# TianmingQiu/BNN_KFAC

Measured on AMD Instinct MI355X. Metric: images/sec for full KFAC factor pass + factor inversion, MNIST MLP, 1/2/4/8 GPUs, higher is better.
Workload: dtype f32; 1 GPU; C2: MLP 784-128-10 KFAC factor pass over 60000 images/rank (batch 4096/rank, global batch 4096) + invert(0.04000000000000001, 200); global_batch=4096, images_per_rank=60000, parallelism=dp1

## Files before the change

### bnn_kfac_amd/_native.py

```python
from __future__ import annotations

import atexit
import ctypes
import os
import threading

import torch

_HERE = os.path.dirname(os.path.abspath(__file__))
LIB_PATH = os.environ.get("BNN_KFAC_AMD_LIB", os.path.join(_HERE, "libkfac_hip.so"))

KFAC_OK, KFAC_EINVAL, KFAC_ELAUNCH, KFAC_EWORKSPACE = 0, -1, -2, -3
ROWMAJOR, CHANNEL, PATCH = 0, 1, 2
OUT_INV_CHOL, OUT_INVERSE = 0, 1
TRI_SYMMETRIC, TRI_LOWER = 0, 1
(PROF_FACTOR_TILES, PROF_FACTOR_REDUCE, PROF_INVERT, PROF_QUAD_TILES, PROF_FACTOR_SYRK3,
 PROF_FACTOR_X3, PROF_FACTOR_CONV, PROF_FACTOR_CHANNEL_SMALL, PROF_SYEV, PROF_FACTOR_CONV_X3,
 PROF_FACTOR_CONV_X3S, PROF_FACTOR_CONV_X3F, PROF_FACTOR_CHANNEL_X3) = range(13)
PROF_FACTOR_KERNELS = {PROF_FACTOR_TILES: "kfac_factor_tiles", PROF_FACTOR_SYRK3: "kfac_factor_syrk3",
                       PROF_FACTOR_X3: "kfac_factor_tiles_x3", PROF_FACTOR_CONV: "kfac_factor_conv",
                       PROF_FACTOR_CHANNEL_SMALL: "kfac_factor_channel_small",
                       PROF_FACTOR_CONV_X3: "kfac_factor_conv_x3", PROF_FACTOR_CONV_X3S: "kfac_factor_conv_x3s",
                       PROF_FACTOR_CONV_X3F: "kfac_factor_conv_x3f", PROF_FACTOR_CHANNEL_X3: "kfac_factor_channel_x3"}

# ... 74 lines not shown


class CovOuterFullJob(ctypes.Structure):
    _fields_ = [("a", c_vp), ("lda", c_i64), ("cols", c_i32), ("has_ones", c_i32), ("D", c_vp),
                ("ldD", c_i64), ("nG", c_i32), ("reserved", c_i32), ("VA", c_vp), ("ldA", c_i64),
                ("VG", c_vp), ("ldG", c_i64), ("W", c_vp), ("ldW", c_i64)]


class InfCovJob(ctypes.Structure):
    _fields_ = [("J", c_vp), ("ldJ", c_i64), ("nA", c_i32), ("nG", c_i32), ("UA", c_vp),
                ("ldA", c_i64), ("ra", c_i32), ("UG", c_vp), ("ldG", c_i64), ("rg", c_i32),
                ("W", c_vp), ("ldW", c_i64), ("F", c_vp), ("ldF", c_i64)]


class InfCovOuterJob(ctypes.Structure):
    _fields_ = [("a", c_vp), ("lda", c_i64), ("cols", c_i32), ("has_ones", c_i32), ("D", c_vp),
                ("ldD", c_i64), ("nG", c_i32), ("reserved", c_i32), ("UA", c_vp), ("ldA", c_i64),
                ("ra", c_i32), ("UG", c_vp), ("ldG", c_i64), ("rg", c_i32), ("W", c_vp),
                ("ldW", c_i64), ("F", c_vp), ("ldF", c_i64)]


class SampleJob(ctypes.Structure):
    _fields_ = [("LA", c_vp), ("ldA", c_i64), ("LG", c_vp), ("ldG", c_i64), ("Z", c_vp),
                ("nA", c_i32), ("nG", c_i32), ("W", c_vp), ("ldW", c_i64), ("bias", c_vp),
                ("wcols", c_i32), ("dense", c_i32)]


class EfbJob(ctypes.Structure):
    _fields_ = [("VA", c_vp), ("ldA", c_i64), ("VG", c_vp), ("ldG", c_i64), ("grad", c_vp),
                ("ld_grad", c_i64), ("state", c_vp), ("ld_state", c_i64), ("diag", c_vp),
                ("ld_diag", c_i64), ("nA", c_i32), ("nG", c_i32), ("accumulate", c_i32),
                ("scale", c_f32)]


class GramJob(ctypes.Structure):
    _fields_ = [("UA", c_vp), ("ldA", c_i64), ("UG", c_vp), ("ldG", c_i64), ("c", c_vp),
                ("sigma", c_vp), ("out", c_vp), ("ldo", c_i64), ("nA", c_i32), ("nG", c_i32),
                ("la", c_i32), ("lg", c_i32)]


class TriJob(ctypes.Structure):
    _fields_ = [("F", c_vp), ("ldF", c_i64), ("n", c_i32), ("reserved", c_i32), ("offset", c_i64)]


SIGNATURES = {
    "kfac_factor_workspace_bytes": (ctypes.c_size_t, [ctypes.POINTER(FactorJob), ctypes.c_int]),
    "kfac_factor_update": (ctypes.c_int, [ctypes.POINTER(FactorJob), ctypes.c_int, c_vp,
                                          ctypes.c_size_t, c_vp]),
    "kfac_factor_accum_plan": (ctypes.c_int, [ctypes.POINTER(FactorJob), ctypes.c_int,
                                              ctypes.POINTER(c_i32), ctypes.POINTER(ctypes.c_size_t)]),
    "kfac_factor_route": (ctypes.c_int, [ctypes.POINTER(FactorJob), ctypes.c_int, ctypes.POINTER(c_i32)]),
    "kfac_factor_flush": (ctypes.c_int, [ctypes.POINTER(FactorJob), ctypes.c_int, c_vp]),
    "kfac_x3_unit_table": (ctypes.c_int, [ctypes.c_int, ctypes.POINTER(c_i32), ctypes.c_int]),
    "kfac_syrk_linear": (ctypes.c_int, [c_vp, c_i64, c_i64, c_i64, ctypes.c_int, c_f32, c_f32,
                                        c_vp, c_i64, c_vp, ctypes.c_size_t, c_vp]),
    "kfac_syrk_conv": (ctypes.c_int, [c_vp, c_i64] + [ctypes.c_int] * 10 + [c_f32, c_f32, c_vp,
                                                                            c_i64, c_vp,
                                                                            ctypes.c_size_t, c_vp]),
    "kfac_syrk_convgrad": (ctypes.c_int, [c_vp, c_i64, ctypes.c_int, c_i64, c_f32, c_f32, c_vp,
                                          c_i64, c_vp, ctypes.c_size_t, c_vp]),
    "kfac_invert_workspace_bytes": (ctypes.c_size_t, [ctypes.POINTER(InvertJob), ctypes.c_int]),
    "kfac_invert": (ctypes.c_int, [ctypes.POINTER(InvertJob), ctypes.c_int, c_vp,
                                   ctypes.c_size_t, c_vp, c_vp]),
    "kfac_invert_ex": (ctypes.c_int, [ctypes.POINTER(InvertJob), ctypes.c_int, c_vp,
                                      ctypes.c_size_t, c_vp, c_vp, c_vp]),
    "kfac_damped_inv_chol": (ctypes.c_int, [c_vp, ctypes.c_int, c_i64, c_f64, c_f64, c_vp, c_i64,
                                            c_vp, ctypes.c_size_t, c_vp, c_vp]),
    "kfac_eig_workspace_bytes": (ctypes.c_size_t, [ctypes.POINTER(EigJob), ctypes.c_int]),
    "kfac_syev": (ctypes.c_int, [ctypes.POINTER(EigJob), ctypes.c_int, c_vp, ctypes.c_size_t,
                                 c_vp, c_vp]),
    "kfac_quadform_workspace_bytes": (ctypes.c_size_t, [ctypes.POINTER(QuadJob), ctypes.c_int,
                                                        c_i64]),
    "kfac_kron_quadform": (ctypes.c_int, [ctypes.POINTER(QuadJob), ctypes.c_int, c_i64,
                                          ctypes.c_int, c_vp, c_vp, ctypes.c_size_t, c_vp]),
    "kfac_kron_cov_workspace_bytes": (ctypes.c_size_t, [ctypes.POINTER(CovJob), ctypes.c_int, c_i64,
                                                        ctypes.c_int]),
    "kfac_kron_cov": (ctypes.c_int, [ctypes.POINTER(CovJob), ctypes.c_int, c_i64, ctypes.c_int,
                                     ctypes.c_int, c_vp, c_vp, ctypes.c_size_t, c_vp]),
    "kfac_kron_cov_outer_workspace_bytes": (ctypes.c_size_t, [ctypes.POINTER(CovOuterJob), ctypes.c_int,
                                                              c_i64, ctypes.c_int]),
    "kfac_kron_cov_outer": (ctypes.c_int, [ctypes.POINTER(CovOuterJob), ctypes.c_int, c_i64, ctypes.c_int,
                                           ctypes.c_int, c_vp, c_vp, ctypes.c_size_t, c_vp]),
    "kfac_cov_conv_rows": (ctypes.c_int, [ctypes.POINTER(CovConvRowsJob), ctypes.c_int, c_i64, ctypes.c_int,
                                          c_vp]),
    "kfac_kron_cov_joint_workspace_bytes": (ctypes.c_size_t, [ctypes.POINTER(CovJob), ctypes.c_int, c_i64,
                                                              ctypes.c_int]),
    "kfac_kron_cov_joint": (ctypes.c_int, [ctypes.POINTER(CovJob), ctypes.c_int, c_i64, ctypes.c_int,
                                           ctypes.c_int, c_vp, c_i64, c_vp, ctypes.c_size_t, c_vp]),
    "kfac_kron_cov_outer_joint_workspace_bytes": (ctypes.c_size_t, [ctypes.POINTER(CovOuterJob),
                                                                    ctypes.c_int, c_i64, ctypes.c_int]),
    "kfac_kron_cov_outer_joint": (ctypes.c_int, [ctypes.POINTER(CovOuterJob), ctypes.c_int, c_i64,
                                                 ctypes.c_int, ctypes.c_int, c_vp, c_i64, c_vp,
                                                 ctypes.c_size_t, c_vp]),
    "kfac_kron_cov_tiled_workspace_bytes": (ctypes.c_size_t, [ctypes.POINTER(CovJob), ctypes.c_int, c_i64,
                                                              ctypes.c_int]),
    "kfac_kron_cov_tiled": (ctypes.c_int, [ctypes.POINTER(CovJob), ctypes.c_int, c_i64, ctypes.c_int,
                                           ctypes.c_int, c_vp, c_vp, ctypes.c_size_t, c_vp]),
    "kfac_kron_cov_outer_tiled_workspace_bytes": (ctypes.c_size_t, [ctypes.POINTER(CovOuterJob),
                                                                    ctypes.c_int, c_i64, ctypes.c_int]),
    "kfac_kron_cov_outer_tiled": (ctypes.c_int, [ctypes.POINTER(CovOuterJob), ctypes.c_int, c_i64,
                                                 ctypes.c_int, ctypes.c_int, c_vp, c_vp, ctypes.c_size_t,
                                                 c_vp]),
    "kfac_glm_draws_workspace_bytes": (ctypes.c_size_t, [ctypes.POINTER(DrawJob), ctypes.c_int, c_i64,
                                                         ctypes.c_int, c_i64]),
    "kfac_glm_draws": (ctypes.c_int, [ctypes.POINTER(DrawJob), ctypes.c_int, c_i64, ctypes.c_int, c_i64,
                                      ctypes.c_int, c_vp, c_i64, c_vp, ctypes.c_size_t, c_vp]),
# ... 767 lines not shown
```

### bnn_kfac_amd/csrc/factor.hip

```cpp
#include <algorithm>
#include <utility>
#include <vector>

#include "factor_common.h"

namespace kfac {

struct Plan {
  int tiles, splits;
  int units;
  int tasks;
  int64_t chunk;
  size_t slab_bytes;
};

static int factor_n(const kfac_factor_job& j) { return j.x.cols + (j.x.has_ones ? 1 : 0); }

static int64_t job_sps(const kfac_factor_job& j) { return std::max<int64_t>(1, cdiv(j.x.rows, BK)); }
static int job_nseg(const kfac_factor_job& j) { return j.nseg > 1 ? j.nseg : 1; }
static bool job_ragged(const kfac_factor_job& j) {
  return j.nseg > 1 && j.x.last_rows > 0 && j.x.last_rows < j.x.rows;
}
static int64_t job_stages(const kfac_factor_job& j) {
  if (job_ragged(j)) return job_sps(j) * (j.nseg - 1) + std::max<int64_t>(1, cdiv(j.x.last_rows, BK));
// ... 236 lines not shown
    d.rdelta = (int)(jb.x.rows - jb.x.last_rows);
    d.rstage = (int64_t)d.sps * (jb.nseg - 1);
    d.rw = (float)((double)jb.x.rows / (double)jb.x.last_rows);
    d.rinv = (float)((double)jb.x.last_rows / (double)jb.x.rows);
  }
}

struct GroupLaunch {
  FactorArgs args, red;
  int tasks, rtiles;
};

static int prepare_group(const kfac_factor_job* jobs, int njobs, const Route& route, char* ws,
                         size_t ws_bytes, GroupLaunch& g) {
  Plan plans[MAXJ];
  plan_jobs(jobs, njobs, route, plans);
  FactorArgs& args = g.args;
  FactorArgs& red = g.red;
  args = FactorArgs{};
  red = FactorArgs{};
  args.njobs = njobs;
  args.split_major = 1;
  int tasks = 0, rtiles = 0, nsegs = 0;
  size_t off = 0;
  for (int i = 0; i < njobs; ++i) {
    const kfac_factor_job& jb = jobs[i];
    FactorJobDev& d = args.job[i];
    fill_dev(d, jb);
    d.glds = job_glds(jb);
    d.x3units = route.family == KFAC_PROF_FACTOR_X3 ? plans[i].units : 0;
    d.splits = plans[i].splits;
    d.sstride = jb.acc && jb.acc_stride > 0 ? jb.acc_stride : d.splits;
    d.chunk = plans[i].chunk;
    if (d.nseg > 1) {
      const float* const* bases = reinterpret_cast<const float* const*>(jb.seg_ptrs);
      d.seg_off = nsegs;
      for (int s = 0; s < d.nseg; ++s) args.segs[nsegs++] = bases[s];
    }
    if (jb.acc) {
      d.slab = jb.acc;
    } else {
      d.slab = reinterpret_cast<float*>(ws + off);
      off += plans[i].slab_bytes;
      FactorJobDev& e = red.job[red.njobs];
      e = d;
      e.tile_begin = rtiles;
      rtiles += plans[i].tiles;
      red.tile_end[red.njobs++] = rtiles;
    }
    d.task_begin = tasks;
    tasks += plans[i].tasks;
    args.task_end[i] = tasks;
  }
  g.tasks = tasks;
  g.rtiles = rtiles;
  return off > ws_bytes ? KFAC_EWORKSPACE : KFAC_OK;
}

static int factor_group(const kfac_factor_job* jobs, int njobs, const Route& route, char* ws,
                        size_t ws_bytes, hipStream_t stream) {
  GroupLaunch g;
  const int rc = prepare_group(jobs, njobs, route, ws, ws_bytes, g);
  if (rc != KFAC_OK) return rc;
  if (g.tasks == 0) return KFAC_OK;
  {
    double work = 0.0, bytes = 0.0;
    if (prof_on())
      for (int i = 0; i < njobs; ++i) {
        work += (double)job_krows(jobs[i]) * factor_n(jobs[i]) * (factor_n(jobs[i]) + 1);
        bytes += job_operand_bytes(jobs[i]);
      }
    ProfScope ps(route.family, stream, work, bytes);
    const int lrc = family_of(route).launch(g.args, route.cg, g.tasks, stream);
    if (lrc != KFAC_OK) return lrc;
    KFAC_CHECK_LAUNCH();
  }
  launch_reduce(g.red, g.rtiles, stream);
  KFAC_CHECK_LAUNCH();
  return KFAC_OK;
}

static size_t group_ws(const kfac_factor_job* jobs, int njobs, const Route& route) {
  Plan plans[MAXJ];
  plan_jobs(jobs, njobs, route, plans);
  size_t off = 0;
  for (int i = 0; i < njobs; ++i) off += plans[i].slab_bytes;
  return off;
}

}

using namespace kfac;

static void launch_groups(const kfac_factor_job* jobs, int njobs, std::vector<kfac_factor_job>& sorted,
                          std::vector<int>& order, std::vector<std::pair<int, int>>& groups) {
  sorted.clear();
  order.clear();
  groups.clear();
  for (int i = 0; i < njobs; ++i)
    if (jobs[i].x.layout == KFAC_ROWMAJOR) {
      sorted.push_back(jobs[i]);
      order.push_back(i);
    }
  const int nrm = (int)sorted.size();
  for (int g = 0; g < nrm; g += MAXJ) groups.emplace_back(g, std::min(MAXJ, nrm - g));
  for (int i = 0; i < njobs; ++i)
// ... 263 lines not shown
```

### bnn_kfac_amd/csrc/factor_common.h

```cpp
#pragma once

#include <cstddef>

#include "kfac_common.h"

namespace kfac {

constexpr int MAXJ = 16;
constexpr int KSEG = 64;

struct FactorJobDev {
  OpDev x;
  float alpha, beta;
  float* F;
  int64_t ldF;
  float* slab;
  int seg_off;
  int64_t chunk;
  int64_t nst;
  int sps, nseg;
  int n, t, splits;
  int task_begin;
  int glds;
  int tile_begin;
// ... 10 lines not shown
struct FactorArgs {
  const float* segs[KSEG];
  int njobs;
  int split_major;
  int task_end[MAXJ];
  int tile_end[MAXJ];
  FactorJobDev job[MAXJ];
};

template <class At>
__device__ __forceinline__ void put_partial(const FactorJobDev& J, const floatx16& acc, At at) {
  if (!J.accum) {
#pragma unroll
    for (int v = 0; v < 16; ++v) *at(v) = acc[v];
    return;
  }
  if (J.sbeta == 0.f) {
#pragma unroll
    for (int v = 0; v < 16; ++v) *at(v) = J.alpha * acc[v];
    return;
  }
  float old[16];
#pragma unroll
  for (int v = 0; v < 16; ++v) old[v] = *at(v);
#pragma unroll
  for (int v = 0; v < 16; ++v) *at(v) = fmaf(J.sbeta, old[v], J.alpha * acc[v]);
}

template <int N, class At>
__device__ __forceinline__ void load_partials(const FactorJobDev& J, int nb, float (&old)[N][16], At at) {
  if (!J.accum || J.sbeta == 0.f) return;
#pragma unroll
  for (int i = 0; i < N; ++i) {
    if (i >= nb) break;
#pragma unroll
    for (int v = 0; v < 16; ++v) old[i][v] = *at(i, v);
  }
}
template <int N, class At>
__device__ __forceinline__ void put_partials(const FactorJobDev& J, int nb, const floatx16 (&acc)[N],
                                             const float (&old)[N][16], At at) {
  const bool upd = J.accum && J.sbeta != 0.f;
  const float a = J.accum ? J.alpha : 1.f;
#pragma unroll
  for (int i = 0; i < N; ++i) {
    if (i >= nb) break;
#pragma unroll
    for (int v = 0; v < 16; ++v) *at(i, v) = upd ? fmaf(J.sbeta, old[i][v], a * acc[i][v]) : a * acc[i][v];
  }
}

__device__ __forceinline__ const float* seg_base(const FactorJobDev& J, const float* const* segs,
                                                 int seg) {
  return J.seg_off >= 0 ? segs[J.seg_off + seg] : J.x.ptr;
}

__device__ __forceinline__ int64_t seg_rows(const FactorJobDev& J, int seg) {
  return J.x.rows - (int64_t)(seg == J.nseg - 1) * J.rdelta;
}

template <int NA>
__device__ __forceinline__ void scale_acc(floatx16 (&acc)[NA], float f) {
#pragma unroll
  for (int a = 0; a < NA; ++a)
#pragma unroll
    for (int v = 0; v < 16; ++v) acc[a][v] *= f;
}

struct StageCursor {
  int seg;
  int64_t k;
  __device__ __forceinline__ void init(const FactorJobDev& J, int64_t s) {
    seg = (int)(s / J.sps);
    k = (s - (int64_t)seg * J.sps) * BK;
  }
  __device__ __forceinline__ void next(int64_t rows) {
    k += BK;
    if (k >= rows) { k = 0; ++seg; }
  }
};

template <int NW = 4>
__device__ __forceinline__ void store_narrow(const FactorJobDev& J, float* out, floatx16& acc,
                                             float* lds) {
  const int lane = threadIdx.x & 63, wave = threadIdx.x >> 6;
  __syncthreads();
  if (wave > 0) {
#pragma unroll
    for (int v = 0; v < 16; ++v) lds[((wave - 1) * 16 + v) * 64 + lane] = acc[v];
  }
  __syncthreads();
  if (wave != 0) return;
#pragma unroll
  for (int w = 0; w < NW - 1; ++w)
#pragma unroll
    for (int v = 0; v < 16; ++v) acc[v] += lds[(w * 16 + v) * 64 + lane];
  put_partial(J, acc, [&](int v) { return &out[acc_row(v, lane) * TILE + (lane & 31)]; });
}

template <int NW = 4>
__device__ __forceinline__ void narrow_direct_load(const FactorJobDev& J, const float* base, int64_t k0,
                                                   int64_t rows, float (&v)[BK / (2 * NW)]) {
  const int lane = threadIdx.x & 63, wave = threadIdx.x >> 6, rr = lane & 31, h = lane >> 5;
#pragma unroll
  for (int s2 = 0; s2 < BK / (2 * NW); ++s2) {
    const int64_t k = k0 + 2 * (wave * (BK / (2 * NW)) + s2) + h;
    v[s2] = k < rows ? (rr < J.x.cols ? base[k * J.x.ld + rr] : (rr == J.x.ones ? 1.f : 0.f)) : 0.f;
// ... 60 lines not shown
  int Wp;
  int ones_base;
  int zero_base;
  int lds;
  int src;
  int nq;
  int units;
  int nb;
  int L;
  int Wo, sh, sw;
  int LPC;
  int nch;
  int pitch;
  int imgf;
  int ones;
  int ldsb;
  int kw;
  int xs_ncopy;
  int xs_hp;
  int xs_pw;
  int xs_cs;
  int xs_g8;
  int xs_grp;
  int xs_np;
  int xs_wp2;
  int xf_nv;
  int xf_vmap;
  int xf_one, xf_zero, xf_dummy;
  int xf_nks;
  int xf_wave[4];
  int xs_lb[32];
  int8_t xs_f[32];
  int xf_cb[128];
};


static inline int raise_dynamic_lds(const void* kernel, int bytes) {
  return hipFuncSetAttribute(kernel, hipFuncAttributeMaxDynamicSharedMemorySize, bytes) == hipSuccess
             ? KFAC_OK : KFAC_ELAUNCH;
}

constexpr int TILES_WGS = 4;
int launch_tiles(const FactorArgs& args, int tasks, hipStream_t stream);
void launch_reduce(const FactorArgs& red, int tiles, hipStream_t stream);

constexpr int S3D_WGS = 2;
int64_t syrk3_units(int n);
int launch_syrk3(const FactorArgs& args, int tasks, hipStream_t stream);

constexpr int X3_WGS = 4;
constexpr int X3_PMAX = 64;
constexpr int X3_UCAP = 2048;
constexpr uint32_t X3_DIAG = 1u << 28;
struct X3Units {
  uint32_t u[X3_UCAP];
};
__host__ __device__ inline int x3_unit_np(uint32_t u) { return (int)(u >> 24) & 7; }
__host__ __device__ inline int x3_unit_panel(uint32_t u, int s) { return (int)(u >> (6 * s)) & 63; }
static inline int x3_panels(int n) { return (n + 31) / 32; }
int x3_unit_table(int P, const uint32_t** table);
int x3_units(int n);
int x3_table_entries(const int* n, int njobs);
int launch_tiles_x3(const FactorArgs& args, int tasks, hipStream_t stream);

constexpr int KFAC_CONV_OCC = 4;
bool conv_fp32_geom(const kfac_operand& o, ConvGeom& g);
int launch_conv(const FactorArgs& args, const ConvGeom& g, int tasks, hipStream_t stream);

constexpr int CONV_X3_WGS = 1;
bool conv_x3_geom(const kfac_operand& o, ConvGeom& g);
int launch_conv_x3(const FactorArgs& args, const ConvGeom& g, int tasks, hipStream_t stream);
bool conv_x3s_geom(const kfac_operand& o, ConvGeom& g);
int launch_conv_x3s(const FactorArgs& args, const ConvGeom& g, int tasks, hipStream_t stream);
bool conv_x3f_geom(const kfac_operand& o, ConvGeom& g);
int launch_conv_x3f(const FactorArgs& args, const ConvGeom& g, int tasks, hipStream_t stream);

constexpr int CHANNEL_WGS = 4;
bool channel_small(const ConvGeom& g);
bool channel_x3_geom(const kfac_operand& o, ConvGeom& g);
int launch_channel_x3(const FactorArgs& args, const ConvGeom& g, int tasks, hipStream_t stream);
int launch_channel_small(const FactorArgs& args, const ConvGeom& g, int tasks, hipStream_t stream);

}
```

### bnn_kfac_amd/csrc/factor_tiles_x3.hip

```cpp
#include <algorithm>
#include <mutex>
#include <type_traits>
#include <vector>

#include "bf16x3.h"
#include "factor_common.h"

namespace kfac {

constexpr int X3_THREADS = 128;

constexpr int X3_NW = X3_THREADS / 64;

struct X3Col {
  int voff;
  bool fill;
  float fv;
};

__device__ __forceinline__ void x3_load8(float (&x)[8], __amdgpu_buffer_rsrc_t rs, const X3Col& c,
                                         int sbase, int sstep) {
#pragma unroll
  for (int r = 0; r < 8; ++r)
    x[r] = __uint_as_float(__builtin_amdgcn_raw_buffer_load_b32(rs, c.voff, sbase + r * sstep, 0));
}

struct X3Cursor {
  const float* b;
  int seg, k;
};

template <int NV>
__device__ __forceinline__ void x3_pattern() {
#pragma unroll
  for (int i = 0; i < 6; ++i) {
    __builtin_amdgcn_sched_group_barrier(0x008, 1, 0);
    if (NV > 0) __builtin_amdgcn_sched_group_barrier(0x002, NV, 0);
    if (i < 4) __builtin_amdgcn_sched_group_barrier(0x020, 2, 0);
  }
}

constexpr int X3_KDIAG = 0;
constexpr int X3_NACC = 6;
__host__ __device__ constexpr int x3_kind_blocks(int kind) { return kind == X3_KDIAG ? 4 : kind * (kind - 1) / 2; }

template <int KIND, bool FILL>
__device__ __forceinline__ void x3_loop(const FactorJobDev& J, const float* const* segs, const int (&pn)[4],
                                        int64_t s0, int64_t s1, floatx16 (&acc)[x3_kind_blocks(KIND)]) {
  constexpr bool DIAG = KIND == X3_KDIAG;
  constexpr int NP = DIAG ? 4 : KIND;
  static_assert(NP >= 2 && NP <= 4, "a unit has two to four panel slots");
  const int lane = threadIdx.x & 63;
  const int wave = __builtin_amdgcn_readfirstlane(threadIdx.x >> 6);
  const int ld4 = (int)J.x.ld * 4;
  const int rows = (int)J.x.rows;
  const int rec = rows * ld4;
  const int rec_last = rec - J.rdelta * ld4;
  const int lr = 16 * wave + 8 * (lane >> 5);
  int voff[4];
  bool onesl[4];
#pragma unroll
  for (int f = 0; f < 4; ++f) {
    const int c = pn[f] * 32 + (lane & 31);
    voff[f] = c < J.x.cols ? lr * ld4 + c * 4 : rec;
    onesl[f] = c == J.x.ones;
  }
  const int ns = (int)(s1 - s0);
  const int lastseg = J.nseg - 1;
  X3Cursor c2;
  c2.seg = (int)(s0 / J.sps);
  c2.k = (int)((s0 - (int64_t)c2.seg * J.sps) * BK);
  c2.b = seg_base(J, segs, c2.seg);
  const float* nb = seg_base(J, segs, min(c2.seg + 1, lastseg));
  int left = ns - 1;
  auto advance = [&](X3Cursor& c) {
    const bool more = left > 0;
    const bool wrap = more && c.k + BK >= rows;
    c.k = more ? (wrap ? 0 : c.k + BK) : c.k;
    c.seg += wrap;
    c.b = wrap ? nb : c.b;
    nb = seg_base(J, segs, min(c.seg + 1, lastseg));
    left -= more;
  };
  auto rsrc = [&](const float* b, int seg) {
    return __builtin_amdgcn_make_buffer_rsrc(const_cast<float*>(b), 0, seg == lastseg ? rec_last : rec,
                                             0x00020000);
  };
  auto ld8 = [&](int f, const X3Cursor& c, float (&x)[8]) {
    x3_load8(x, rsrc(c.b, c.seg), X3Col{voff[f], false, 0.f}, c.k * ld4, ld4);
  };
  float x[4][8];
  const int k0 = c2.k, seg0 = c2.seg;
#pragma unroll
  for (int f = 0; f < NP; ++f) ld8(f, c2, x[f]);
  advance(c2);
  X3Cursor c1 = c2;
  int kc = k0, kcs = seg0;
  auto take = [&](int f, int kstage, int kseg, const X3Cursor& c) {
    X3Frag fr = x3_split8(x[f]);
    if (FILL && (DIAG || f == NP - 1)) {
      typedef uint32_t u32x4 __attribute__((ext_vector_type(4)));
      const int nv = onesl[f] ? (int)seg_rows(J, kseg) - kstage - lr : 0;
      u32x4 h = __builtin_bit_cast(u32x4, fr.p[0]);
#pragma unroll
      for (int i = 0; i < 4; ++i) h[i] |= (nv > 2 * i ? 0x3f80u : 0u) | (nv > 2 * i + 1 ? 0x3f800000u : 0u);
      fr.p[0] = __builtin_bit_cast(bf16x8, h);
    }
    ld8(f, c, x[f]);
    return fr;
  };
  X3Frag pa = take(0, k0, seg0, c2);
  X3Frag pb = take(1, k0, seg0, c2);
  asm volatile("s_waitcnt vmcnt(0)" ::: "memory");
  constexpr int NV = FILL ? 52 / 6 + 1 : 44 / 6 + 1;
  auto stage = [&](const X3Frag& F0, const X3Frag& F1, X3Frag& F0n, X3Frag& F1n) {
    const int kn = c2.k, kns = c2.seg;
    c1 = c2;
    advance(c2);
    __builtin_amdgcn_sched_barrier(0);
    if constexpr (DIAG) {
      const X3Frag F2 = take(2, kc, kcs, c1);
      x3_six(acc[0], F0, F0);
      x3_pattern<NV>();
      __builtin_amdgcn_sched_barrier(0);
      const X3Frag F3 = take(3, kc, kcs, c1);
      x3_six(acc[1], F1, F1);
      x3_pattern<NV>();
      __builtin_amdgcn_sched_barrier(0);
      F0n = take(0, kn, kns, c2);
      x3_six(acc[2], F2, F2);
      x3_pattern<NV>();
      __builtin_amdgcn_sched_barrier(0);
      F1n = take(1, kn, kns, c2);
      x3_six(acc[3], F3, F3);
      x3_pattern<NV>();
    } else if constexpr (NP == 4) {
      const X3Frag F2 = take(2, kc, kcs, c1);
      x3_six(acc[0], F1, F0);
      x3_pattern<NV>();
      __builtin_amdgcn_sched_barrier(0);
      const X3Frag F3 = take(3, kc, kcs, c1);
      x3_six(acc[1], F2, F0);
      x3_pattern<NV>();
      __builtin_amdgcn_sched_barrier(0);
      x3_six(acc[3], F3, F0);
      x3_pattern<0>();
      __builtin_amdgcn_sched_barrier(0);
      F0n = take(0, kn, kns, c2);
      x3_six(acc[2], F2, F1);
      x3_pattern<NV>();
      __builtin_amdgcn_sched_barrier(0);
      x3_six(acc[4], F3, F1);
      x3_pattern<0>();
      __builtin_amdgcn_sched_barrier(0);
      F1n = take(1, kn, kns, c2);
      x3_six(acc[5], F3, F2);
      x3_pattern<NV>();
    } else if constexpr (NP == 3) {
      const X3Frag F2 = take(2, kc, kcs, c1);
      x3_six(acc[0], F1, F0);
      x3_pattern<NV>();
      __builtin_amdgcn_sched_barrier(0);
      F0n = take(0, kn, kns, c2);
      x3_six(acc[1], F2, F0);
      x3_pattern<NV>();
      __builtin_amdgcn_sched_barrier(0);
      F1n = take(1, kn, kns, c2);
      x3_six(acc[2], F2, F1);
      x3_pattern<NV>();
    } else {
      F0n = take(0, kn, kns, c2);
      F1n = take(1, kn, kns, c2);
      x3_six(acc[0], F1, F0);
      x3_pattern<2 * NV>();
    }
    kc = kn;
    kcs = kns;
  };
  const int64_t rst = J.rstage;
  const int bst = (rst > s0 && rst < s1) ? (int)(rst - s0) : -1;
  for (int st = 0; st < ns; ++st) {
    if (st == bst) scale_acc(acc, J.rinv);
    X3Frag qa, qb;
    stage(pa, pb, qa, qb);
    pa = qa;
    pb = qb;
  }
  if (rst >= 0 && s1 > rst) scale_acc(acc, J.rw);
}

template <int KIND>
__device__ __forceinline__ void x3_unit(const FactorJobDev& J, const float* const* segs, const int (&pn)[4],
                                        int np, int split, float* lds) {
  constexpr bool DIAG = KIND == X3_KDIAG;
  constexpr int NB = x3_kind_blocks(KIND);
  const int64_t s0 = (int64_t)split * J.chunk;
  const int64_t s1 = min(J.nst, s0 + J.chunk);
  const int lane = threadIdx.x & 63;
  const int wave = __builtin_amdgcn_readfirstlane(threadIdx.x >> 6);
  floatx16 acc[NB];
#pragma unroll
  for (int b = 0; b < NB; ++b)
#pragma unroll
    for (int v = 0; v < 16; ++v) acc[b][v] = 0.f;
  if (s1 > s0) {
    const int op = J.x.ones >> 5;
    const bool fill = J.x.ones >= 0 && (pn[0] == op || pn[1] == op || pn[2] == op || pn[3] == op);
    if (fill) x3_loop<KIND, true>(J, segs, pn, s0, s1, acc);
    else x3_loop<KIND, false>(J, segs, pn, s0, s1, acc);
  }
  const int nblk = DIAG ? np : NB;
  constexpr int HALF = (NB + 1) / 2;
  __syncthreads();
#pragma unroll
  for (int b = 0; b < NB; ++b) {
    const bool mine = (b < HALF) == (wave == 0);
    if (b < nblk && !mine)
#pragma unroll
      for (int v = 0; v < 16; ++v) lds[(b * 16 + v) * 64 + lane] = acc[b][v];
  }
  __syncthreads();
#pragma unroll
  for (int b = 0; b < NB; ++b) {
    const bool mine = (b < HALF) == (wave == 0);
    if (b >= nblk || !mine) continue;
    constexpr int BI[6] = {1, 2, 2, 3, 3, 3}, BJ[6] = {0, 0, 1, 0, 1, 2};
    const int pr = DIAG ? pn[b & 3] : pn[BI[b]], pc = DIAG ? pn[b & 3] : pn[BJ[b]];
    const int ti = pr >> 1, tj = pc >> 1;
    float* out = J.slab + ((size_t)(ti * (ti + 1) / 2 + tj) * J.sstride + split) * TILE * TILE +
                 (pr & 1) * 32 * TILE + (pc & 1) * 32;
#pragma unroll
    for (int v = 0; v < 16; ++v) acc[b][v] += lds[(b * 16 + v) * 64 + lane];
    put_partial(J, acc[b], [&](int v) { return &out[acc_row(v, lane) * TILE + (lane & 31)]; });
  }
}

template <int GBK>
__device__ __forceinline__ void factor_task_x3(const FactorJobDev& J, const float* const* segs,
                                               const X3Units& U, int local, float* lds, int split_major) {
  static_assert(GBK == 16 * X3_NW, "one 16-row half stage per wave");
  const int units = J.x3units;
  const int split = split_major ? local / units : local % J.splits;
  const int unit = split_major ? local - split * units : local / J.splits;
  const uint32_t u = U.u[J.x3tab + unit];
  const int np = x3_unit_np(u);
  const int pn[4] = {x3_unit_panel(u, 0), x3_unit_panel(u, 1), x3_unit_panel(u, 2), x3_unit_panel(u, 3)};
  switch ((u & X3_DIAG) ? X3_KDIAG : np) {
    case 4: x3_unit<4>(J, segs, pn, np, split, lds); break;
    case 3: x3_unit<3>(J, segs, pn, np, split, lds); break;
    case 2: x3_unit<2>(J, segs, pn, np, split, lds); break;
    case X3_KDIAG: x3_unit<X3_KDIAG>(J, segs, pn, np, split, lds); break;
    default: break;
  }
}

__global__ __launch_bounds__(X3_THREADS, 2) void kfac_factor_tiles_x3(FactorArgs args, X3Units units) {
  __shared__ __attribute__((aligned(16))) float lds[X3_NACC * 16 * 64];
  const int task = xcd_task(blockIdx.x, gridDim.x);
  int j = 0;
  while (j + 1 < args.njobs && task >= args.task_end[j]) ++j;
  const int local = task - args.job[j].task_begin;
  const FactorJobDev& J = args.job[j];
  if (J.n <= 32)
    factor_task_narrow_direct<X3_NW>(J, args.segs, local, lds);
  else
    factor_task_x3<BK>(J, args.segs, units, local, lds, args.split_major);
}

namespace {

uint32_t x3_pack(const int* p, int np, bool diag) {
  uint32_t u = (uint32_t)np << 24 | (diag ? X3_DIAG : 0u);
  for (int s = 0; s < 4; ++s) u |= (uint32_t)p[std::min(s, np - 1)] << (6 * s);
  return u;
}

std::vector<uint32_t> x3_build_table(int P) {
  std::vector<uint32_t> k4, k3, k2, dg;
  std::vector<char> used((size_t)P * P, 0);
  auto is_free = [&](int a, int b) { return !used[(size_t)a * P + b]; };
  auto mark = [&](int a, int b) { used[(size_t)a * P + b] = used[(size_t)b * P + a] = 1; };
  if (P == 25) {
    const int base[4][2] = {{0, 0}, {0, 1}, {1, 0}, {2, 2}};
    for (int m = 1; m <= 2; ++m)
      for (int sx = 0; sx < 5; ++sx)
        for (int sy = 0; sy < 5; ++sy) {
          int p[4];
          for (int i = 0; i < 4; ++i) p[i] = 5 * ((m * base[i][0] + sx) % 5) + (m * base[i][1] + sy) % 5;
          std::sort(p, p + 4);
          for (int i = 0; i < 4; ++i)
            for (int j = 0; j < i; ++j) mark(p[i], p[j]);
          k4.push_back(x3_pack(p, 4, false));
        }
  }
  for (int a = 0; a < P; ++a)
    for (int b = a + 1; b < P; ++b) {
      if (!is_free(a, b)) continue;
      for (int c = b + 1; c < P && is_free(a, b); ++c) {
        if (!is_free(a, c) || !is_free(b, c)) continue;
        for (int d = c + 1; d < P; ++d)
          if (is_free(a, d) && is_free(b, d) && is_free(c, d)) {
            const int p[4] = {a, b, c, d};
            for (int i = 0; i < 4; ++i)
              for (int j = 0; j < i; ++j) mark(p[i], p[j]);
            k4.push_back(x3_pack(p, 4, false));
            break;
          }
      }
    }
  for (int a = 0; a < P; ++a)
    for (int b = a + 1; b < P; ++b)
      for (int c = b + 1; c < P && is_free(a, b); ++c)
        if (is_free(a, c) && is_free(b, c)) {
          const int p[3] = {a, b, c};
          mark(a, b), mark(a, c), mark(b, c);
          k3.push_back(x3_pack(p, 3, false));
        }
  for (int a = 0; a < P; ++a)
    for (int b = a + 1; b < P; ++b)
      if (is_free(a, b)) {
        const int p[2] = {a, b};
        mark(a, b);
        k2.push_back(x3_pack(p, 2, false));
      }
  for (int a = 0; a < P; a += 4) {
    int p[4], np = 0;
    for (; np < 4 && a + np < P; ++np) p[np] = a + np;
    dg.push_back(x3_pack(p, np, true));
  }
  std::vector<uint32_t> t(k4);
  t.insert(t.end(), dg.begin(), dg.end());
  t.insert(t.end(), k3.begin(), k3.end());
  t.insert(t.end(), k2.begin(), k2.end());
  return t;
}

}

int x3_unit_table(int P, const uint32_t** table) {
  static std::mutex mu;
  static std::vector<uint32_t> tables[X3_PMAX + 1];
  if (P < 2 || P > X3_PMAX) return 0;
  std::lock_guard<std::mutex> lock(mu);
  if (tables[P].empty()) tables[P] = x3_build_table(P);
  if (table) *table = tables[P].data();
  return (int)tables[P].size();
}

int x3_units(int n) { return n <= 32 ? 1 : x3_unit_table(x3_panels(n), nullptr); }

int x3_table_entries(const int* n, int njobs) {
  bool seen[X3_PMAX + 1] = {};
  int total = 0;
  for (int i = 0; i < njobs; ++i) {
    const int P = x3_panels(n[i]);
    if (n[i] <= 32 || P > X3_PMAX || seen[P]) continue;
    seen[P] = true;
    total += x3_unit_table(P, nullptr);
  }
  return total;
}

int launch_tiles_x3(const FactorArgs& args, int tasks, hipStream_t stream) {
  FactorArgs a = args;
  X3Units U;
  int off[X3_PMAX + 1], total = 0;
  std::fill(off, off + X3_PMAX + 1, -1);
  for (int i = 0; i < a.njobs; ++i) {
    FactorJobDev& d = a.job[i];
    d.x3tab = 0;
    if (d.n <= 32) continue;
    const int P = x3_panels(d.n);
    const uint32_t* t = nullptr;
    const int nu = x3_unit_table(P, &t);
    if (nu == 0 || nu != d.x3units) return KFAC_ELAUNCH;
    if (off[P] < 0) {
      if (total + nu > X3_UCAP) return KFAC_ELAUNCH;
      std::copy(t, t + nu, U.u + total);
      off[P] = total;
      total += nu;
    }
    d.x3tab = off[P];
  }
  std::fill(U.u + total, U.u + X3_UCAP, 0u);
  hipLaunchKernelGGL(kfac_factor_tiles_x3, dim3(tasks), dim3(X3_THREADS), 0, stream, a, U);
  return KFAC_OK;
}

}

extern "C" int kfac_x3_unit_table(int P, int32_t* out, int cap) {
  const uint32_t* t = nullptr;
  const int nu = kfac::x3_unit_table(P, &t);
  for (int i = 0; i < nu && i < cap && out; ++i) {
    const int np = kfac::x3_unit_np(t[i]);
    const bool diag = (t[i] & kfac::X3_DIAG) != 0;
    for (int s = 0; s < 4; ++s) out[6 * i + s] = s < np ? kfac::x3_unit_panel(t[i], s) : -1;
    out[6 * i + 4] = diag ? 0 : (np == 4 ? 63 : np == 3 ? 0b001011 : 0b000001);
    out[6 * i + 5] = diag ? (1 << np) - 1 : 0;
  }
  return nu;
}
```

### bnn_kfac_amd/csrc/kfac_common.h

```cpp
#pragma once

#include <hip/hip_runtime.h>
#include <stdint.h>

#include "../../include/kfac_hip.h"
#include "knobs.h"

namespace kfac {

constexpr int TILE = 64;
constexpr int BK = 32;
constexpr int LDP = TILE + 1;
constexpr int NTHREADS = 256;
constexpr int PANEL = BK * (TILE + 4);
constexpr int IMAXJ = 8;

typedef float floatx16 __attribute__((ext_vector_type(16)));

#define KFAC_CHECK_LAUNCH()                                   \
  do {                                                        \
    if (hipGetLastError() != hipSuccess) return KFAC_ELAUNCH; \
  } while (0)

static inline int64_t cdiv(int64_t a, int64_t b) { return (a + b - 1) / b; }
// ... 188 lines not shown
  const int lane = tid & 63, wave = tid >> 6;
  const int qi = narrow ? 0 : wave >> 1, qj = narrow ? 0 : wave & 1;
  const int h = lane >> 5, rr = lane & 31;

  Panel<LA> pa;
  Panel<LB> pb;
  pa.init(opA, base ? base : opA.ptr, i0, tid, k1, k0);
  pb.init(opB, base ? base : opB.ptr, j0, tid, k1, k0);
  float va[8], vb[8];

  pa.load(k0, va);
  if (!same) pb.load(k0, vb);
  pa.store(lds, va);
  if (!same) pb.store(lds + PANEL, vb);
  __syncthreads();

  int cur = 0;
  for (int64_t k = k0; k < k1; k += BK) {
    const bool more = k + BK < k1;
    if (more) {
      pa.load(k + BK, va);
      if (!same) pb.load(k + BK, vb);
    }
    float* bcur = lds + 2 * cur * PANEL;
    const float* a = bcur + h * Panel<LA>::PITCH + qi * 32 + rr;
    const float* b = bcur + (same ? 0 : PANEL) + h * Panel<LB>::PITCH + qj * 32 + rr;
    if (narrow) {
#pragma unroll
      for (int s = 0; s < BK / 8; ++s) {
        const int ks = 2 * (wave * (BK / 8) + s);
        acc = __builtin_amdgcn_mfma_f32_32x32x2f32(a[ks * Panel<LA>::PITCH], b[ks * Panel<LB>::PITCH],
                                                   acc, 0, 0, 0);
      }
    } else if (active) {
#pragma unroll
      for (int s = 0; s < BK / 2; ++s)
        acc = __builtin_amdgcn_mfma_f32_32x32x2f32(a[2 * s * Panel<LA>::PITCH],
                                                   b[2 * s * Panel<LB>::PITCH], acc, 0, 0, 0);
    }
    if (more) {
      float* bnext = lds + 2 * (cur ^ 1) * PANEL;
      pa.store(bnext, va);
      if (!same) pb.store(bnext + PANEL, vb);
    }
    __syncthreads();
    cur ^= 1;
  }
}

__device__ __forceinline__ int acc_row(int v, int lane) {
  return (v & 3) + 8 * (v >> 2) + 4 * (lane >> 5);
}

__device__ __forceinline__ int xcd_task(int b, int n) {
  const int x = b & 7, s = b >> 3, per = n >> 3, rem = n & 7;
  return (x < rem ? x * (per + 1) : rem * (per + 1) + (x - rem) * per) + s;
}

__device__ __forceinline__ void tri_decode(int t, int& ti, int& tj) {
  int i = (int)((sqrtf(8.f * (float)t + 1.f) - 1.f) * 0.5f);
  while ((i + 1) * (i + 2) / 2 <= t) ++i;
  while (i * (i + 1) / 2 > t) --i;
  ti = i;
  tj = t - i * (i + 1) / 2;
}

}
```

### include/kfac_hip.h

```cpp
#ifndef KFAC_HIP_H
#define KFAC_HIP_H

#include <stddef.h>
#include <stdint.h>

#ifdef __cplusplus
extern "C" {
#endif

#if defined(__GNUC__) || defined(__clang__)
#define KFAC_API __attribute__((visibility("default")))
#else
#define KFAC_API
#endif

typedef void* kfac_stream_t;

enum kfac_status {
  KFAC_OK = 0,
  KFAC_EINVAL = -1,
  KFAC_ELAUNCH = -2,
  KFAC_EWORKSPACE = -3,
};

enum kfac_layout { KFAC_ROWMAJOR = 0, KFAC_CHANNEL = 1, KFAC_PATCH = 2 };

typedef struct kfac_operand {
  const float* ptr;
  int32_t layout;
  int32_t cols;
  int64_t rows;
  int32_t has_ones;
  int32_t last_rows;
  int64_t ld;
  int64_t L;
  int64_t sB;
  int32_t C, H, W, kh, kw, sh, sw, ph, pw, Ho, Wo, reserved1;
} kfac_operand;

typedef struct kfac_factor_job {
  kfac_operand x;
  float alpha;
  float beta;
  float* F;
  int64_t ldF;
  float* acc;
  int32_t acc_splits;
  float acc_beta;
  const void* seg_ptrs;
  int32_t nseg;
  int32_t acc_stride;
} kfac_factor_job;

KFAC_API size_t kfac_factor_workspace_bytes(const kfac_factor_job* jobs, int njobs);
KFAC_API int kfac_factor_update(const kfac_factor_job* jobs, int njobs, void* workspace,
                       size_t workspace_bytes, kfac_stream_t stream);

KFAC_API int kfac_factor_accum_plan(const kfac_factor_job* jobs, int njobs, int32_t* splits,
                           size_t* bytes);
KFAC_API int kfac_factor_route(const kfac_factor_job* jobs, int njobs, int32_t* family);
KFAC_API int kfac_factor_flush(const kfac_factor_job* jobs, int njobs, kfac_stream_t stream);

KFAC_API int kfac_x3_unit_table(int P, int32_t* out, int cap);

KFAC_API int kfac_syrk_linear(const float* x, int64_t B, int64_t d, int64_t ldx, int has_ones,
                     float alpha, float beta, float* F, int64_t ldF, void* workspace,
                     size_t workspace_bytes, kfac_stream_t stream);
KFAC_API int kfac_syrk_conv(const float* x, int64_t B, int C, int H, int W, int kh, int kw, int sh,
                   int sw, int ph, int pw, int has_ones, float alpha, float beta, float* F,
                   int64_t ldF, void* workspace, size_t workspace_bytes, kfac_stream_t stream);
KFAC_API int kfac_syrk_convgrad(const float* g, int64_t B, int C, int64_t L, float alpha, float beta,
                       float* F, int64_t ldF, void* workspace, size_t workspace_bytes,
                       kfac_stream_t stream);

enum kfac_inv_out { KFAC_OUT_INV_CHOL = 0, KFAC_OUT_INVERSE = 1 };

typedef struct kfac_invert_job {
  const float* F;
  int64_t ldF;
  int32_t n;
  int32_t out_kind;
  double scale;
  double shift;
  float* out;
  int64_t ldo;
} kfac_invert_job;

KFAC_API size_t kfac_invert_workspace_bytes(const kfac_invert_job* jobs, int njobs);
KFAC_API int kfac_invert(const kfac_invert_job* jobs, int njobs, void* workspace, size_t workspace_bytes,
                int32_t* info, kfac_stream_t stream);
KFAC_API int kfac_invert_ex(const kfac_invert_job* jobs, int njobs, void* workspace,
                   size_t workspace_bytes, int32_t* info, void* inputs_read, kfac_stream_t stream);
KFAC_API int kfac_damped_inv_chol(const float* F, int n, int64_t ldF, double sqrt_s, double sqrt_n,
                         float* L, int64_t ldL, void* workspace, size_t workspace_bytes,
                         int32_t* info, kfac_stream_t stream);

typedef struct kfac_eig_job {
  const float* F;
  int64_t ldF;
  int32_t n;
  int32_t reserved;
  double* evals;
  float* evecs;
  int64_t ldv;
} kfac_eig_job;

KFAC_API size_t kfac_eig_workspace_bytes(const kfac_eig_job* jobs, int njobs);
KFAC_API int kfac_syev(const kfac_eig_job* jobs, int njobs, void* workspace, size_t workspace_bytes,
              int32_t* info, kfac_stream_t stream);

typedef struct kfac_quad_job {
  const float* J;
  int64_t ldJ;
  int32_t nA, nG;
  const float* K1;
  int64_t ld1;
// ... 359 lines not shown
```

Before: 212.2 million images/s.

## Add mixed off-diagonal/diagonal x3 units and split-major cross-job task ordering

```diff
diff --git a/bnn_kfac_amd/_native.py b/bnn_kfac_amd/_native.py
--- a/bnn_kfac_amd/_native.py
+++ b/bnn_kfac_amd/_native.py
@@ -150,6 +150,8 @@
     "kfac_factor_route": (ctypes.c_int, [ctypes.POINTER(FactorJob), ctypes.c_int, ctypes.POINTER(c_i32)]),
     "kfac_factor_flush": (ctypes.c_int, [ctypes.POINTER(FactorJob), ctypes.c_int, c_vp]),
     "kfac_x3_unit_table": (ctypes.c_int, [ctypes.c_int, ctypes.POINTER(c_i32), ctypes.c_int]),
+    "kfac_x3_task_decode": (ctypes.c_int, [ctypes.POINTER(c_i32), ctypes.c_int, ctypes.c_int, ctypes.c_int,
+                                           ctypes.c_int, ctypes.POINTER(c_i32)]),
     "kfac_syrk_linear": (ctypes.c_int, [c_vp, c_i64, c_i64, c_i64, ctypes.c_int, c_f32, c_f32,
                                         c_vp, c_i64, c_vp, ctypes.c_size_t, c_vp]),
     "kfac_syrk_conv": (ctypes.c_int, [c_vp, c_i64] + [ctypes.c_int] * 10 + [c_f32, c_f32, c_vp,
diff --git a/bnn_kfac_amd/csrc/factor.hip b/bnn_kfac_amd/csrc/factor.hip
--- a/bnn_kfac_amd/csrc/factor.hip
+++ b/bnn_kfac_amd/csrc/factor.hip
@@ -312,6 +312,19 @@
     tasks += plans[i].tasks;
     args.task_end[i] = tasks;
   }
+  if (route.family == KFAC_PROF_FACTOR_X3) {
+    bool same = true;
+    for (int i = 1; i < njobs; ++i) same &= args.job[i].splits == args.job[0].splits;
+    if (same && args.job[0].splits > 0) {
+      args.split_major = 2;
+      int units = 0;
+      for (int i = 0; i < njobs; ++i) {
+        args.job[i].task_begin = units;
+        units += args.job[i].x3units;
+        args.task_end[i] = units;
+      }
+    }
+  }
   g.tasks = tasks;
   g.rtiles = rtiles;
   return off > ws_bytes ? KFAC_EWORKSPACE : KFAC_OK;
diff --git a/bnn_kfac_amd/csrc/factor_common.h b/bnn_kfac_amd/csrc/factor_common.h
--- a/bnn_kfac_amd/csrc/factor_common.h
+++ b/bnn_kfac_amd/csrc/factor_common.h
@@ -86,7 +86,9 @@
 
 __device__ __forceinline__ const float* seg_base(const FactorJobDev& J, const float* const* segs,
                                                  int seg) {
-  return J.seg_off >= 0 ? segs[J.seg_off + seg] : J.x.ptr;
+  const float* queued = segs[max(J.seg_off, 0) + seg];
+  const float* single = J.x.ptr;
+  return J.seg_off >= 0 ? queued : single;
 }
 
 __device__ __forceinline__ int64_t seg_rows(const FactorJobDev& J, int seg) {
@@ -253,12 +255,24 @@
 constexpr int X3_PMAX = 64;
 constexpr int X3_UCAP = 2048;
 constexpr uint32_t X3_DIAG = 1u << 28;
+constexpr int X3_MIX_S3D3 = 1, X3_MIX_P1D2 = 2;
 struct X3Units {
   uint32_t u[X3_UCAP];
 };
 __host__ __device__ inline int x3_unit_np(uint32_t u) { return (int)(u >> 24) & 7; }
 __host__ __device__ inline int x3_unit_panel(uint32_t u, int s) { return (int)(u >> (6 * s)) & 63; }
+__host__ __device__ inline int x3_unit_mix(uint32_t u) { return (int)(u >> 29) & 3; }
 static inline int x3_panels(int n) { return (n + 31) / 32; }
+__host__ __device__ __forceinline__ void x3_task_decode(const int* unit_end, int njobs, int splits,
+                                                        int blocks, int block, int& job, int& unit, int& split) {
+  const int U = blocks / splits;
+  const int t = xcd_task(block, blocks);
+  split = t / U;
+  const int lu = t - split * U;
+  job = 0;
+  while (job + 1 < njobs && lu >= unit_end[job]) ++job;
+  unit = lu - (job > 0 ? unit_end[job - 1] : 0);
+}
 int x3_unit_table(int P, const uint32_t** table);
 int x3_units(int n);
 int x3_table_entries(const int* n, int njobs);
diff --git a/bnn_kfac_amd/csrc/factor_tiles_x3.hip b/bnn_kfac_amd/csrc/factor_tiles_x3.hip
--- a/bnn_kfac_amd/csrc/factor_tiles_x3.hip
+++ b/bnn_kfac_amd/csrc/factor_tiles_x3.hip
@@ -40,15 +40,30 @@
   }
 }
 
-constexpr int X3_KDIAG = 0;
+constexpr int X3_KDIAG = 0, X3_KS3D3 = 5, X3_KP1D2 = 6;
 constexpr int X3_NACC = 6;
-__host__ __device__ constexpr int x3_kind_blocks(int kind) { return kind == X3_KDIAG ? 4 : kind * (kind - 1) / 2; }
+__host__ __device__ constexpr int x3_kind_slots(int kind) {
+  return kind == X3_KDIAG || kind == X3_KS3D3 ? 4 : kind == X3_KP1D2 ? 2 : kind;
+}
+__host__ __device__ constexpr int x3_kind_blocks(int kind) {
+  return kind == X3_KDIAG ? 4 : kind == X3_KS3D3 ? 6 : kind == X3_KP1D2 ? 3 : kind * (kind - 1) / 2;
+}
+struct X3Block {
+  int i, j;
+};
+__host__ __device__ constexpr X3Block x3_kind_block(int kind, int b) {
+  constexpr int BI[6] = {1, 2, 2, 3, 3, 3}, BJ[6] = {0, 0, 1, 0, 1, 2};
+  if (kind == X3_KDIAG) return {b & 3, b & 3};
+  if (kind == X3_KS3D3) return b < 3 ? X3Block{3, b} : X3Block{b - 3, b - 3};
+  if (kind == X3_KP1D2) return b == 0 ? X3Block{1, 0} : X3Block{b - 1, b - 1};
+  return {BI[b], BJ[b]};
+}
 
 template <int KIND, bool FILL>
 __device__ __forceinline__ void x3_loop(const FactorJobDev& J, const float* const* segs, const int (&pn)[4],
                                         int64_t s0, int64_t s1, floatx16 (&acc)[x3_kind_blocks(KIND)]) {
   constexpr bool DIAG = KIND == X3_KDIAG;
-  constexpr int NP = DIAG ? 4 : KIND;
+  constexpr int NP = x3_kind_slots(KIND);
   static_assert(NP >= 2 && NP <= 4, "a unit has two to four panel slots");
   const int lane = threadIdx.x & 63;
   const int wave = __builtin_amdgcn_readfirstlane(threadIdx.x >> 6);
@@ -134,6 +149,39 @@
       F1n = take(1, kn, kns, c2);
       x3_six(acc[3], F3, F3);
       x3_pattern<NV>();
+    } else if constexpr (KIND == X3_KS3D3) {
+      const X3Frag F3 = take(3, kc, kcs, c1);
+      x3_six(acc[3], F0, F0);
+      x3_pattern<NV>();
+      __builtin_amdgcn_sched_barrier(0);
+      const X3Frag F2 = take(2, kc, kcs, c1);
+      x3_six(acc[0], F3, F0);
+      x3_pattern<NV>();
+      __builtin_amdgcn_sched_barrier(0);
+      F0n = take(0, kn, kns, c2);
+      x3_six(acc[4], F1, F1);
+      x3_pattern<NV>();
+      __builtin_amdgcn_sched_barrier(0);
+      x3_six(acc[1], F3, F1);
+      x3_pattern<0>();
+      __builtin_amdgcn_sched_barrier(0);
+      F1n = take(1, kn, kns, c2);
+      x3_six(acc[5], F2, F2);
+      x3_pattern<NV>();
+      __builtin_amdgcn_sched_barrier(0);
+      x3_six(acc[2], F3, F2);
+      x3_pattern<0>();
+    } else if constexpr (KIND == X3_KP1D2) {
+      F0n = take(0, kn, kns, c2);
+      x3_six(acc[0], F1, F0);
+      x3_pattern<NV>();
+      __builtin_amdgcn_sched_barrier(0);
+      F1n = take(1, kn, kns, c2);
+      x3_six(acc[1], F0, F0);
+      x3_pattern<NV>();
+      __builtin_amdgcn_sched_barrier(0);
+      x3_six(acc[2], F1, F1);
+      x3_pattern<0>();
     } else if constexpr (NP == 4) {
       const X3Frag F2 = take(2, kc, kcs, c1);
       x3_six(acc[0], F1, F0);
@@ -224,8 +272,8 @@
   for (int b = 0; b < NB; ++b) {
     const bool mine = (b < HALF) == (wave == 0);
     if (b >= nblk || !mine) continue;
-    constexpr int BI[6] = {1, 2, 2, 3, 3, 3}, BJ[6] = {0, 0, 1, 0, 1, 2};
-    const int pr = DIAG ? pn[b & 3] : pn[BI[b]], pc = DIAG ? pn[b & 3] : pn[BJ[b]];
+    const X3Block blk = x3_kind_block(KIND, b);
+    const int pr = pn[blk.i], pc = pn[blk.j];
     const int ti = pr >> 1, tj = pc >> 1;
     float* out = J.slab + ((size_t)(ti * (ti + 1) / 2 + tj) * J.sstride + split) * TILE * TILE +
                  (pr & 1) * 32 * TILE + (pc & 1) * 32;
@@ -237,47 +285,53 @@
 
 template <int GBK>
 __device__ __forceinline__ void factor_task_x3(const FactorJobDev& J, const float* const* segs,
-                                               const X3Units& U, int local, float* lds, int split_major) {
+                                               const X3Units& U, int unit, int split, float* lds) {
   static_assert(GBK == 16 * X3_NW, "one 16-row half stage per wave");
-  const int units = J.x3units;
-  const int split = split_major ? local / units : local % J.splits;
-  const int unit = split_major ? local - split * units : local / J.splits;
   const uint32_t u = U.u[J.x3tab + unit];
-  const int np = x3_unit_np(u);
+  const int np = x3_unit_np(u), mix = x3_unit_mix(u);
   const int pn[4] = {x3_unit_panel(u, 0), x3_unit_panel(u, 1), x3_unit_panel(u, 2), x3_unit_panel(u, 3)};
-  switch ((u & X3_DIAG) ? X3_KDIAG : np) {
+  switch (mix == X3_MIX_S3D3 ? X3_KS3D3 : mix == X3_MIX_P1D2 ? X3_KP1D2 : (u & X3_DIAG) ? X3_KDIAG : np) {
     case 4: x3_unit<4>(J, segs, pn, np, split, lds); break;
     case 3: x3_unit<3>(J, segs, pn, np, split, lds); break;
     case 2: x3_unit<2>(J, segs, pn, np, split, lds); break;
     case X3_KDIAG: x3_unit<X3_KDIAG>(J, segs, pn, np, split, lds); break;
+    case X3_KS3D3: x3_unit<X3_KS3D3>(J, segs, pn, np, split, lds); break;
+    case X3_KP1D2: x3_unit<X3_KP1D2>(J, segs, pn, np, split, lds); break;
     default: break;
   }
 }
 
 __global__ __launch_bounds__(X3_THREADS, 2) void kfac_factor_tiles_x3(FactorArgs args, X3Units units) {
   __shared__ __attribute__((aligned(16))) float lds[X3_NACC * 16 * 64];
-  const int task = xcd_task(blockIdx.x, gridDim.x);
-  int j = 0;
-  while (j + 1 < args.njobs && task >= args.task_end[j]) ++j;
-  const int local = task - args.job[j].task_begin;
+  int j = 0, unit, split;
+  if (args.split_major == 2) {
+    x3_task_decode(args.task_end, args.njobs, args.job[0].splits, gridDim.x, blockIdx.x, j, unit, split);
+  } else {
+    const int task = xcd_task(blockIdx.x, gridDim.x);
+    while (j + 1 < args.njobs && task >= args.task_end[j]) ++j;
+    const int local = task - args.job[j].task_begin;
+    const int nu = args.job[j].x3units, ns = args.job[j].splits;
+    split = args.split_major ? local / nu : local % ns;
+    unit = args.split_major ? local - split * nu : local / ns;
+  }
   const FactorJobDev& J = args.job[j];
   if (J.n <= 32)
-    factor_task_narrow_direct<X3_NW>(J, args.segs, local, lds);
+    factor_task_narrow_direct<X3_NW>(J, args.segs, split, lds);
   else
-    factor_task_x3<BK>(J, args.segs, units, local, lds, args.split_major);
+    factor_task_x3<BK>(J, args.segs, units, unit, split, lds);
 }
 
 namespace {
 
-uint32_t x3_pack(const int* p, int np, bool diag) {
-  uint32_t u = (uint32_t)np << 24 | (diag ? X3_DIAG : 0u);
+uint32_t x3_pack(const int* p, int np, bool diag, int mix = 0) {
+  uint32_t u = (uint32_t)np << 24 | (diag ? X3_DIAG : 0u) | (uint32_t)mix << 29;
   for (int s = 0; s < 4; ++s) u |= (uint32_t)p[std::min(s, np - 1)] << (6 * s);
   return u;
 }
 
 std::vector<uint32_t> x3_build_table(int P) {
-  std::vector<uint32_t> k4, k3, k2, dg;
-  std::vector<char> used((size_t)P * P, 0);
+  std::vector<uint32_t> k4, s3, k3, p1, k2, dg;
+  std::vector<char> used((size_t)P * P, 0), dused(P, 0);
   auto is_free = [&](int a, int b) { return !used[(size_t)a * P + b]; };
   auto mark = [&](int a, int b) { used[(size_t)a * P + b] = used[(size_t)b * P + a] = 1; };
   if (P == 25) {
@@ -316,21 +370,45 @@
           mark(a, b), mark(a, c), mark(b, c);
           k3.push_back(x3_pack(p, 3, false));
         }
+  for (int h = 0; h < P; ++h) {
+    int p[4], np = 0;
+    for (int a = 0; a < h; ++a) {
+      if (!is_free(a, h) || dused[a]) continue;
+      p[np++] = a;
+      if (np < 3) continue;
+      p[3] = h;
+      for (int i = 0; i < 3; ++i) mark(p[i], h), dused[p[i]] = 1;
+      s3.push_back(x3_pack(p, 4, false, X3_MIX_S3D3));
+      np = 0;
+    }
+  }
   for (int a = 0; a < P; ++a)
-    for (int b = a + 1; b < P; ++b)
-      if (is_free(a, b)) {
-        const int p[2] = {a, b};
-        mark(a, b);
+    for (int b = a + 1; b < P; ++b) {
+      if (!is_free(a, b)) continue;
+      const int p[2] = {a, b};
+      mark(a, b);
+      if (!dused[a] && !dused[b]) {
+        dused[a] = dused[b] = 1;
+        p1.push_back(x3_pack(p, 2, false, X3_MIX_P1D2));
+      } else {
         k2.push_back(x3_pack(p, 2, false));
       }
-  for (int a = 0; a < P; a += 4) {
+    }
+  {
     int p[4], np = 0;
-    for (; np < 4 && a + np < P; ++np) p[np] = a + np;
-    dg.push_back(x3_pack(p, np, true));
+    for (int a = 0; a < P; ++a) {
+      if (!dused[a]) p[np++] = a;
+      if (np == 4 || (np > 0 && a == P - 1)) {
+        dg.push_back(x3_pack(p, np, true));
+        np = 0;
+      }
+    }
   }
   std::vector<uint32_t> t(k4);
+  t.insert(t.end(), s3.begin(), s3.end());
   t.insert(t.end(), dg.begin(), dg.end());
   t.insert(t.end(), k3.begin(), k3.end());
+  t.insert(t.end(), p1.begin(), p1.end());
   t.insert(t.end(), k2.begin(), k2.end());
   return t;
 }
@@ -395,9 +473,32 @@
   for (int i = 0; i < nu && i < cap && out; ++i) {
     const int np = kfac::x3_unit_np(t[i]);
     const bool diag = (t[i] & kfac::X3_DIAG) != 0;
+    const int mix = kfac::x3_unit_mix(t[i]);
     for (int s = 0; s < 4; ++s) out[6 * i + s] = s < np ? kfac::x3_unit_panel(t[i], s) : -1;
-    out[6 * i + 4] = diag ? 0 : (np == 4 ? 63 : np == 3 ? 0b001011 : 0b000001);
-    out[6 * i + 5] = diag ? (1 << np) - 1 : 0;
+    out[6 * i + 4] = mix == kfac::X3_MIX_S3D3 ? 0b110100 : mix == kfac::X3_MIX_P1D2 ? 0b000001
+                     : diag ? 0 : (np == 4 ? 63 : np == 3 ? 0b001011 : 0b000001);
+    out[6 * i + 5] = mix == kfac::X3_MIX_S3D3 ? 0b0111 : mix == kfac::X3_MIX_P1D2 ? 0b0011
+                     : diag ? (1 << np) - 1 : 0;
   }
   return nu;
 }
+
+extern "C" int kfac_x3_task_decode(const int32_t* units, int njobs, int splits, int blocks, int block,
+                                   int32_t* xcd_job_unit_split) {
+  if (!units || !xcd_job_unit_split || njobs < 1 || njobs > kfac::MAXJ || splits < 1) return KFAC_EINVAL;
+  int64_t U = 0;
+  int unit_end[kfac::MAXJ];
+  for (int i = 0; i < njobs; ++i) {
+    if (units[i] < 1 || units[i] > kfac::X3_UCAP) return KFAC_EINVAL;
+    U += units[i];
+    unit_end[i] = (int)U;
+  }
+  if (U * splits != blocks || block < 0 || block >= blocks) return KFAC_EINVAL;
+  int job, unit, split;
+  kfac::x3_task_decode(unit_end, njobs, splits, blocks, block, job, unit, split);
+  xcd_job_unit_split[0] = block & 7;
+  xcd_job_unit_split[1] = job;
+  xcd_job_unit_split[2] = unit;
+  xcd_job_unit_split[3] = split;
+  return KFAC_OK;
+}
diff --git a/bnn_kfac_amd/csrc/kfac_common.h b/bnn_kfac_amd/csrc/kfac_common.h
--- a/bnn_kfac_amd/csrc/kfac_common.h
+++ b/bnn_kfac_amd/csrc/kfac_common.h
@@ -264,7 +264,7 @@
   return (v & 3) + 8 * (v >> 2) + 4 * (lane >> 5);
 }
 
-__device__ __forceinline__ int xcd_task(int b, int n) {
+__host__ __device__ __forceinline__ int xcd_task(int b, int n) {
   const int x = b & 7, s = b >> 3, per = n >> 3, rem = n & 7;
   return (x < rem ? x * (per + 1) : rem * (per + 1) + (x - rem) * per) + s;
 }
diff --git a/include/kfac_hip.h b/include/kfac_hip.h
--- a/include/kfac_hip.h
+++ b/include/kfac_hip.h
@@ -62,6 +62,8 @@
 KFAC_API int kfac_factor_flush(const kfac_factor_job* jobs, int njobs, kfac_stream_t stream);
 
 KFAC_API int kfac_x3_unit_table(int P, int32_t* out, int cap);
+KFAC_API int kfac_x3_task_decode(const int32_t* units, int njobs, int splits, int blocks, int block,
+                        int32_t* xcd_job_unit_split);
 
 KFAC_API int kfac_syrk_linear(const float* x, int64_t B, int64_t d, int64_t ldx, int has_ones,
                      float alpha, float beta, float* F, int64_t ldF, void* workspace,
```

Measured after the change: 214.6 million images/s (median of 6 runs). +1.1%, better.
